# FAST-ASR/MarkovModels.jl

Hardware: AMD Instinct MI355X
Metric: pdfposteriors_frames_per_sec (higher is better)
Workload: dtype f32

## Files before the change

### markovmodels.jl_amd/csrc/mm_kernel_pairs.hip

```cpp
#pragma once
#include <algorithm>
#include "mm_internal.h"
#include "mm_kernel_rows.hip"

namespace mm {

typedef float mm_f32x2 __attribute__((ext_vector_type(2)));
typedef unsigned mm_u32x2 __attribute__((ext_vector_type(2)));
__device__ __forceinline__ mm_u32x2 ldsr2u(unsigned addr) { return *(__attribute__((address_space(3))) const mm_u32x2 *)(__UINTPTR_TYPE__)addr; }
__device__ __forceinline__ mm_f32x2 ldsr2(unsigned addr) { return *(__attribute__((address_space(3))) const mm_f32x2 *)(__UINTPTR_TYPE__)addr; }
__device__ __forceinline__ void ldsw2(unsigned addr, float a, float b) {
    mm_f32x2 v = {a, b};
    *(__attribute__((address_space(3))) mm_f32x2 *)(__UINTPTR_TYPE__)addr = v;
}

constexpr int pair_pc(int NJ) { return NJ > 4 ? 64 * NJ : 256; }
constexpr int pair_nr(int RS, int PC) { return (PC > 256 || RS > 16384) ? 2 : 3; }
template <int RS, int PHASE, int RSH = 2 * RS, int PC = 256>
struct PairLay {
    static constexpr unsigned RS2 = 2 * RS;
    static constexpr unsigned PC4 = 4u * PC, PC8 = 8u * PC;
    static constexpr int NR = pair_nr(RS, PC);
    static constexpr unsigned RAWS = 2u * PC4;
    static constexpr unsigned XPS = 2u * PC;
    static constexpr unsigned PP(int par) { return unsigned(par) * RS2; }
    static constexpr unsigned RAW(int k, int u) { return 2 * RS2 + unsigned(2 * k + u) * PC4; }
    static constexpr unsigned EM(int par) { return 2 * RS2 + 8u * PC4 + unsigned(par) * PC8; }
    static constexpr unsigned MS(int par) { return 2 * RS2 + 8u * PC4 + 2u * PC8 + unsigned(par) * 64u; }
    static constexpr unsigned OWN(int k) { return 2 * RS2 + 8u * PC4 + 2u * PC8 + 128u + unsigned(k) * 16u; }
    static constexpr unsigned XFLAG = 2 * RS2 + 8u * PC4 + 2u * PC8 + 192u;
    static constexpr unsigned MX(int par) { return 2 * RS2 + 8u * PC4 + 2u * PC8 + 200u + unsigned(par) * 8u; }
    static constexpr int POFFN = NR == 2 ? 4 : 8;
    static constexpr unsigned POFFB = 16u * POFFN;
    static constexpr unsigned POFF(int k, int u) { return 2 * RS2 + 8u * PC4 + 2u * PC8 + 256u + unsigned(2 * k + u) * 8u; }
    static constexpr unsigned PSUM(int par) { return 2 * RS2 + 8u * PC4 + 2u * PC8 + 256u + POFFB + unsigned(par) * PC8; }
    static constexpr unsigned PDFSE = 2 * RS2 + 8u * PC4 + 4u * PC8 + 256u + POFFB;
    static constexpr unsigned FIX = PDFSE + PC4;
    static constexpr unsigned AL(int k) { return FIX + unsigned(k) * RSH; }
    static constexpr unsigned Q(int par) { return FIX + unsigned(NR) * RSH + unsigned(par) * RSH; }
    static constexpr unsigned SLOTS = PHASE ? FIX + unsigned(NR + 2) * RSH : FIX;
};
inline size_t pair_lds_bytes(int RS, int phase, int nslotrows, int RSH = 0, int PC = 256) {
    const size_t fix = size_t(4 * RS) + size_t(8 * 4 * PC) + size_t(4 * 8 * PC) + 256 + (pair_nr(RS, PC) == 2 ? 64 : 128) + size_t(4 * PC);
    return fix + (phase ? size_t(pair_nr(RS, PC) + 2) * size_t(RSH ? RSH : 2 * RS) : 0) + size_t(nslotrows) * 64 * 8;
}

typedef unsigned long long mm_u64;
typedef __attribute__((address_space(1))) mm_u64 mm_gu64;
#ifndef MM_SPLIT_TIMEOUT
#ifndef MM_PAIR_LINFIN
#define MM_PAIR_LINFIN 1
#endif
#ifndef MM_PAIR_SCAN_BATCH
#define MM_PAIR_SCAN_BATCH 8
#endif
#define MM_LINF_EMIN (-40.f)
#define MM_SPLIT_TIMEOUT 10000000ull
#endif
__device__ __forceinline__ void granule_store(float *base, unsigned byte_off, float a, float b) {
    const mm_u64 v = ((mm_u64)__builtin_bit_cast(unsigned, b) << 32) | __builtin_bit_cast(unsigned, a);
    __hip_atomic_store((mm_gu64 *)(__UINTPTR_TYPE__)(reinterpret_cast<char *>(base) + byte_off), v, __ATOMIC_RELAXED, __HIP_MEMORY_SCOPE_AGENT);
}
__device__ __forceinline__ mm_u64 granule_load(const float *base, unsigned byte_off) {
    return __hip_atomic_load((mm_gu64 *)(__UINTPTR_TYPE__)(reinterpret_cast<const char *>(base) + byte_off), __ATOMIC_RELAXED,
                             __HIP_MEMORY_SCOPE_AGENT);
}
// ... 154 lines not shown
        "v_max_f32_dpp %1, %1, %1 row_mirror row_mask:0xf bank_mask:0xf\n\ts_nop 1"
        : "+v"(a), "+v"(b));
    const int ia = __builtin_bit_cast(int, a), ib = __builtin_bit_cast(int, b);
    const float a0 = __builtin_bit_cast(float, __builtin_amdgcn_readlane(ia, 0)), b0 = __builtin_bit_cast(float, __builtin_amdgcn_readlane(ib, 0));
    const float a1 = __builtin_bit_cast(float, __builtin_amdgcn_readlane(ia, 16)), b1 = __builtin_bit_cast(float, __builtin_amdgcn_readlane(ib, 16));
    const float a2 = __builtin_bit_cast(float, __builtin_amdgcn_readlane(ia, 32)), b2 = __builtin_bit_cast(float, __builtin_amdgcn_readlane(ib, 32));
    const float a3 = __builtin_bit_cast(float, __builtin_amdgcn_readlane(ia, 48)), b3 = __builtin_bit_cast(float, __builtin_amdgcn_readlane(ib, 48));
    a = fmaxf(fmaxf(a0, a1), fmaxf(a2, a3));
    b = fmaxf(fmaxf(b0, b1), fmaxf(b2, b3));
}

__device__ __forceinline__ float wave_max_of2(float a, float b) {
    float v = max_nc(a, b);
    asm("s_nop 1\n\tv_max_f32_dpp %0, %0, %0 quad_perm:[1,0,3,2] row_mask:0xf bank_mask:0xf\n\ts_nop 1\n\t"
        "v_max_f32_dpp %0, %0, %0 quad_perm:[2,3,0,1] row_mask:0xf bank_mask:0xf\n\ts_nop 1\n\t"
        "v_max_f32_dpp %0, %0, %0 row_half_mirror row_mask:0xf bank_mask:0xf\n\ts_nop 1\n\t"
        "v_max_f32_dpp %0, %0, %0 row_mirror row_mask:0xf bank_mask:0xf\n\ts_nop 1\n\t"
        "v_max_f32_dpp %0, %0, %0 row_bcast:15 row_mask:0xa bank_mask:0xf\n\ts_nop 1\n\t"
        "v_max_f32_dpp %0, %0, %0 row_bcast:31 row_mask:0xc bank_mask:0xf\n\ts_nop 1"
        : "+v"(v));
    return __builtin_bit_cast(float, __builtin_amdgcn_readlane(__builtin_bit_cast(int, v), 63));
}

template <int NJ, bool ADAPT>
__device__ __forceinline__ void pair_stage_em2(unsigned dst, unsigned raw0, unsigned raw1, int n, int len0, int len1, int P, int lane, float S0,
                                               float S1, float (&E)[2], float &X, int *mark0, int *mark1) {
    float v0[NJ], v1[NJ];
#pragma unroll
    for (int j = 0; j < NJ; ++j) {
        v0[j] = ldsr(raw0 + 256u * j + 4u * lane);
        v1[j] = ldsr(raw1 + 256u * j + 4u * lane);
    }
    float e0 = MM_NINF, e1 = MM_NINF;
#pragma unroll
    for (int j = 0; j < NJ; ++j) {
        const int q = lane + 64 * j;
        v0[j] = em_value(v0[j], n, len0, P, q);
        v1[j] = em_value(v1[j], n, len1, P, q);
        if (q < P) {
            e0 = max_nc(e0, v0[j]);
            e1 = max_nc(e1, v1[j]);
        }
    }
    wave_max_rl2(e0, e1);
    if (!(e0 > MM_NINF)) e0 = 0.f;
    if (!(e1 > MM_NINF)) e1 = 0.f;
    float n0 = 0.f, n1 = 0.f;
#pragma unroll
    for (int j = 0; j < NJ; ++j) {
        const int q = lane + 64 * j;
        if (q <= P) {
            const float x0 = v0[j] - e0 - S0, x1 = v1[j] - e1 - S1;
            ldsw2(dst + 8u * (unsigned)q, fast_exp2(x0), fast_exp2(x1));
            n0 = max_nc(n0, v0[j] > MM_NINF ? -x0 : 0.f);
            n1 = max_nc(n1, v1[j] > MM_NINF ? -x1 : 0.f);
        }
    }
    if constexpr (ADAPT) {
        X = wave_max_of2(n0, n1);
    } else {
        if (n0 > -MM_LINF_EMIN) *mark0 = 1;
        if (n1 > -MM_LINF_EMIN) *mark1 = 1;
    }
    E[0] = e0;
    E[1] = e1;
}

template <int NJ, bool LIN = false>
__device__ __forceinline__ void pair_stage_em_wide(unsigned dst, unsigned raw0, unsigned raw1, int n, int len0, int len1, int P, int lane,
                                                   float (&E)[2], float S0 = 0.f, float S1 = 0.f, int *mark0 = nullptr, int *mark1 = nullptr) {
    constexpr int NP = (NJ + 3) / 4;
    mm_f32x4 v0[NP], v1[NP];
#pragma unroll
    for (int j = 0; j < NP; ++j) {
        const unsigned o = 4u * (unsigned)(256 * j + 4 * lane);
        v0[j] = *(__attribute__((address_space(3))) const mm_f32x4 *)(__UINTPTR_TYPE__)(raw0 + o);
        v1[j] = *(__attribute__((address_space(3))) const mm_f32x4 *)(__UINTPTR_TYPE__)(raw1 + o);
    }
    float e0 = MM_NINF, e1 = MM_NINF;
#pragma unroll
    for (int j = 0; j < NP; ++j) {
#pragma unroll
        for (int i = 0; i < 4; ++i) {
            const int q = 256 * j + 4 * lane + i;
            v0[j][i] = em_value(v0[j][i], n, len0, P, q);
            v1[j][i] = em_value(v1[j][i], n, len1, P, q);
            if (q < P) {
                e0 = max_nc(e0, v0[j][i]);
// ... 324 lines not shown
#ifndef MM_PAIR_PRIO_A
#define MM_PAIR_PRIO_A 8
#define MM_PAIR_PRIO_B 16
#endif
#define MM_PAIR_PRIO(k, lvl) if constexpr (2 * (k) < KA) __builtin_amdgcn_s_setprio(lvl);
#define MM_PAIR_CASES(M)                                                                                     \
    M(0) M(2) M(4) M(6) MM_PAIR_PRIO(MM_PAIR_PRIO_A, 1) M(8) M(10) M(12)                                     \
    if (lastp >= 14) {                                                                                       \
        M(14) MM_PAIR_PRIO(MM_PAIR_PRIO_B, 0) M(16)                                                          \
        if (lastp >= 18) {                                                                                   \
            M(18)                                                                                            \
            if (lastp >= 20) { M(20) M(22) }                                                                 \
        }                                                                                                    \
    }

struct PairHand {
    float m_prev, s_cur, s_prev, cbar;
    int seen, pad;
    double cum;
};

template <int KA, int RS, int PHASE, int DIRT, int NJ, int H = 1, int RSH = 2 * RS, bool SMALL = false, bool XPT = false>
__device__ __forceinline__ void pair_agent(const RunParams &p, int pair, int hset = 0, int rdir = 0) {
#ifndef MM_SPLIT_MAXTRACK
#define MM_SPLIT_MAXTRACK 0
#endif
    extern __shared__ float lds[];
    const int DIR = DIRT < 0 ? __builtin_amdgcn_readfirstlane(rdir) : DIRT;
    const unsigned long long x_tmo = p.x_timeout;
    using L = PairLay<RS, PHASE, RSH, pair_pc(NJ)>;
#ifndef MM_PAIR_DA
#define MM_PAIR_DA 3
#endif
#ifndef MM_PAIR_DB
#define MM_PAIR_DB 3
#endif
#ifndef MM_PAIR_EXITS_B
#define MM_PAIR_EXITS_B 1
#endif
    constexpr bool MM_PAIR_DOUBLE = true;
    constexpr bool LINF = MM_PAIR_LINFIN != 0 && NJ <= 4;
    constexpr bool ADAPT = LINF && H == 1;
    constexpr int D = PHASE ? MM_PAIR_DB : MM_PAIR_DA;
    const int tid = threadIdx.x, NT = blockDim.x, lane = tid & 63;
    const int wave = __builtin_amdgcn_readfirstlane(tid >> 6), NW = NT >> 6, NWC = NW - (H > 1 ? 2 : 1);
    const bool service = wave == NWC;
    const bool xwave = H > 1 && wave == NWC + 1;
    if (service || xwave) __builtin_amdgcn_s_setprio(3);
    PairUtt U[2];
    int NFp = 1;
#pragma unroll
    for (int u = 0; u < 2; ++u) {
        const int i = 2 * pair + u;
// ... 12 lines not shown
    }
    static_assert(!XPT || PHASE == 0, "the export runs phase A");
    if constexpr (XPT) NFp = p.N + 1;
    float *rowsP = p.ws_alpha + (long long)pair * (long long)(p.N + 2) * 2 * p.pair_s1p;
    const UttDesc &ud = p.utts[U[0].b];
    const RowU r = uni(H > 1 ? ud.rps[DIR][hset] : ud.rp[DIR]);
    const int S1 = r.rows, S1p = p.pair_s1p, P1 = uni(ud.P1), P = P1 - 1, P1p = (P1 + 3) & ~3;
    const float thr = r.thr;
    unsigned sthr = 0u;
    if constexpr (LINF && !ADAPT)
        asm volatile("v_readfirstlane_b32 %0, %1" : "=s"(sthr) : "v"(((unsigned)(127 - (int)(thr + MM_LINF_EMIN < 1.f ? 1.f : thr + MM_LINF_EMIN)) << 23) - 1u));
    int m = (int)(((long long)NFp * (p.split_q10 > 0 ? p.split_q10 : 512)) >> 10);
    m = m < 1 ? 1 : (m > NFp - 1 && NFp > 1 ? NFp - 1 : m);
    const int tA = XPT ? NFp : (DIR ? NFp - m : m), tEnd = NFp;
    auto frame_of = [&](int t) { return DIR ? NFp + 1 - t : t; };
    PairHand *hand = reinterpret_cast<PairHand *>(p.pair_hand) + ((long long)pair * 2 + DIR) * 2;
    if (lds_addr_of(lds) != 0u) __builtin_trap();
    MM_STAMP_DECL;

    for (unsigned q = tid * 4u; q < 2u * L::RS2; q += NT * 4u) ldsw(L::PP(0) + q, 0.f);
    if constexpr (PHASE == 1)
        for (unsigned q = tid * 4u; q < 2u * RSH; q += NT * 4u) ldsw(L::Q(0) + q, 0.f);
    if (tid < 32) ldsw(L::MS(0) + 4u * tid, 0.f);
    if (tid < 4) ldswu(L::MX(0) + 4u * tid, 0u);
    if (tid < 4) ldsw(L::EM(tid >> 1) + 8u * P1p + 4u * (tid & 1), LINF ? 0.f : MM_NINF);
    const int nslotwords = r.nslotrows * 128;
    for (int q = tid; q < nslotwords; q += NT) ldswu(L::SLOTS + 4u * q, as_global(r.slots)[q]);
    if constexpr (PHASE == 1)
        for (int q = tid; q < P1; q += NT) ldswu(L::PDFSE + 4u * q, as_global(reinterpret_cast<const unsigned *>(r.pdfse))[q]);
    int *redo0 = p.redo + U[0].b, *redo1 = p.redo + (U[1].valid ? U[1].b : p.B);
    const int xbase = H > 1 ? p.sp_base[hset] : 0, xcnt = H > 1 ? p.sp_cnt[hset] : 0;
    float *xsend = nullptr, *xps_send = nullptr;
    bool xplain = false;
    const float *xrecv[H], *xps_recv[H];
    if constexpr (H > 1) {
        float *xb = p.xbuf + (long long)PHASE * p.x_phase + ((long long)pair * 2 + DIR) * H * 2 * p.x_slot;
        float *xq = p.xps + ((long long)pair * 2 + DIR) * H * 4 * (int)L::XPS;
#pragma unroll
        for (int g = 0; g < H; ++g) {
            xrecv[g] = g == hset ? nullptr : xb + (long long)g * 2 * p.x_slot;
            xps_recv[g] = g == hset ? nullptr : xq + (long long)g * 4 * (int)L::XPS;
        }
        xsend = xb + (long long)hset * 2 * p.x_slot;
        xps_send = xq + (long long)hset * 4 * (int)L::XPS;
    }
    unsigned long long endmask = 0, lgw0 = 0;
    int nslots = 0, start2 = 0;
// ... 55 lines not shown
#pragma unroll
            for (int u = 0; u < 2; ++u) row_dma_em<NJ>(L::RAW(0, u) + L::RAWS * (unsigned)(t & 3), U[u].Vb, p.vsn, frame_of(tt), p.N, P, sl);
        };
        auto dma_partner = [&](int t) {
            const int tt = t < 1 ? 1 : (t > tEnd ? tEnd : t);
            int f = frame_of(tt);
            f = f > p.N ? p.N : f;
            const int n4 = H > 1 ? (xcnt + 1) >> 1 : S1p >> 1;
            constexpr int NDM = RSH / 1024;
            const mm_f32x4 *src = reinterpret_cast<const mm_f32x4 *>(rowsP + (long long)f * 2 * S1p + 2 * xbase);
            const unsigned dst = L::AL(0) + (unsigned)(tt % L::NR) * (unsigned)RSH;
            if constexpr (small_graph) {
                dma_b128(src + (sl < n4 ? sl : 0), dst);
            } else {
                (void)n4;
                dma_row_b128<NDM>(uni(src), (unsigned)sl, dst);
            }
#pragma unroll
            for (int u = 0; u < 2; ++u)
                if (sl < 2) dma_b32(reinterpret_cast<const unsigned *>(U[u].offs + f) + sl, L::POFF(0, u) + 16u * (unsigned)(t & (L::POFFN - 1)));
        };
        constexpr int NDMA = 2 * NJ + (PHASE ? RSH / 1024 + 2 : 0);
        constexpr int NDMA_SMALL = 2 * NJ + (PHASE ? 1 + 2 : 0);
        auto stage = [&](int t, const float (&S)[2]) {
            float E[2], X = 0.f;
#ifndef MM_PAIR_WIDE_SERVICE
#define MM_PAIR_WIDE_SERVICE 1
#endif
            if constexpr (NJ > 4 && MM_PAIR_WIDE_SERVICE) {
                pair_stage_em_wide<NJ, LINF>(L::EM(t & 1), L::RAW(0, 0) + L::RAWS * (unsigned)(t & 3), L::RAW(0, 1) + L::RAWS * (unsigned)(t & 3), frame_of(t),
                                             U[0].len, U[1].len, P, sl, E, S[0], S[1], redo0, redo1);
            } else if constexpr (LINF) {
                pair_stage_em2<NJ, ADAPT>(L::EM(t & 1), L::RAW(0, 0) + L::RAWS * (unsigned)(t & 3), L::RAW(0, 1) + L::RAWS * (unsigned)(t & 3), frame_of(t),
                                          U[0].len, U[1].len, P, sl, S[0], S[1], E, X, redo0, redo1);
            } else {
#pragma unroll
                for (int u = 0; u < 2; ++u)
                    E[u] = pair_stage_em<NJ, LINF>(L::EM(t & 1), L::RAW(0, u) + L::RAWS * (unsigned)(t & 3), u, frame_of(t), U[u].len, P, sl, S[u], u ? redo1 : redo0);
            }
            double before[2];
#pragma unroll
            for (int u = 0; u < 2; ++u) {
                before[u] = cum[u];
                cum[u] += (double)S[u] + (double)E[u];
            }
            if constexpr (ADAPT) {
                float room = thr_v - X;
                if (room < 16.f) {
                    room = 16.f;
                    if (sl == 0) {
                        *redo0 = 1;
                        *redo1 = 1;
                    }
                }
// ... 21 lines not shown
                norm[u].s_prev = h.s_prev;
                norm[u].cbar = h.cbar;
                norm[u].seen = h.seen;
                cum[u] = h.cum;
            }
        }
        MM_ROW_VMCNT(0);
        if (PHASE == 0 || (DIR == 1 && !LINF)) {
            float E[2];
#pragma unroll
            for (int u = 0; u < 2; ++u) E[u] = pair_stage_em<NJ>(L::EM(t0 & 1), L::RAW(0, u) + L::RAWS * (unsigned)(t0 & 3), u, frame_of(t0), U[u].len, P, sl);
            if (PHASE == 0) {
#pragma unroll
                for (int u = 0; u < 2; ++u) cum[u] = (double)E[u];
                if (DIR == 0 && sl == 0) {
                    U[0].offs[1] = cum[0];
                    U[1].offs[1] = cum[1];
                }
            }
        }
        __syncthreads();
        if (t0 + 1 <= t1) {
            const float S[2] = {norm[0].s_cur, norm[1].s_cur};
            stage(t0 + 1, S);
        }
        dma_raw(t0 + 4);
        __syncthreads();
        const bool gwide = p.gsp == 1 && ((p.gsn | p.gsb) & 1) == 0 && ((__UINTPTR_TYPE__)p.gamma & 7) == 0;
        auto frames_of_step = [&](int ts, unsigned psum) {
            const int f = frame_of(ts);
            const bool live0 = f >= 1 && f <= U[0].len, live1 = f >= 1 && f <= U[1].len;
            float lt[2];
            const float *xp[H];
#pragma unroll
            for (int g = 0; g < H; ++g) xp[g] = (H > 1 && g != hset) ? xps_recv[g] + (ts & 3) * (int)L::XPS : nullptr;
            const bool writer = H == 1 || hset == 0;
            if constexpr (H == 1 && NJ > 4 && MM_PAIR_WIDE_SERVICE) {
                pair_finish_frames_wide<NJ>(psum, P1, P, sl, p.gamma + (long long)U[0].b * p.gsb + (long long)(f - 1) * p.gsn,
                                            p.gamma + (long long)U[1].b * p.gsb + (long long)(f - 1) * p.gsn, p.gsp, live0 && U[0].valid,
                                            live1 && U[1].valid, gwide, lt);
            } else if (!pair_finish_frames<NJ, H>(psum, P1, P, sl, p.gamma + (long long)U[0].b * p.gsb + (long long)(f - 1) * p.gsn,
                                           p.gamma + (long long)U[1].b * p.gsb + (long long)(f - 1) * p.gsn, p.gsp,
                                           live0 && U[0].valid && writer, live1 && U[1].valid && writer, lt, xp, split_tag(ts, t0, 2),
                                           xdead ? 0ull : x_tmo)) {
                if (sl == 0) {
                    *redo0 = 2;
                    *redo1 = 2;
// ... 4 lines not shown
            for (int u = 0; u < 2; ++u)
                if (u ? live1 : live0) {
                    const double own = *(__attribute__((address_space(3))) const double *)(__UINTPTR_TYPE__)(L::OWN(ts & 3) + 8u * u);
                    const double oth = *(__attribute__((address_space(3))) const double *)(__UINTPTR_TYPE__)(L::POFF(0, u) + 16u * (unsigned)(ts & (L::POFFN - 1)));
                    const double z = (double)lt[u] + own + oth;
                    zmin[u] = z < zmin[u] ? z : zmin[u];
                    zmax[u] = z > zmax[u] ? z : zmax[u];
                    if (!(z == z)) zmax[u] = __builtin_inf();
                    ltmin[u] = lt[u] < ltmin[u] ? lt[u] : ltmin[u];
                }
        };
        auto step = [&](auto RDc, int t) {
            constexpr int RD = decltype(RDc)::value, WR = 1 - RD;
#ifndef MM_PAIR_OPAQUE_B
#define MM_PAIR_OPAQUE_B 0
#endif
            if constexpr (H > 1 || NJ > 2 || (MM_PAIR_OPAQUE_B && PHASE == 1)) asm volatile("" : "+v"(sl));
            constexpr bool ring2 = PHASE == 1 && L::NR == 2;
            if constexpr (ring2) dma_partner(t + 1);
            else if constexpr (small_graph) asm volatile("s_waitcnt vmcnt(%0)" ::"n"(NDMA_SMALL) : "memory");
            else asm volatile("s_waitcnt vmcnt(%0)" ::"n"(NDMA) : "memory");
            MM_STAMP(2);
            float mx[2];
            if constexpr (H > 1 && MM_SPLIT_MAXTRACK) {
                if (t == t0 + 1) {
                    pair_scan_max<(RS / 8 + 63) / 64>(L::PP(RD), (S1 + 2) >> 1, sl, mx[0], mx[1]);
                } else {
                    const mm_u32x2 w = ldsr2u(L::MX(RD));
                    mx[0] = fast_log2(__builtin_bit_cast(float, (unsigned)__builtin_amdgcn_readfirstlane((int)w.x)));
                    mx[1] = fast_log2(__builtin_bit_cast(float, (unsigned)__builtin_amdgcn_readfirstlane((int)w.y)));
                }
                if (sl == 0) {
                    ldswu(L::MX(RD), 0u);
                    ldswu(L::MX(RD) + 4u, 0u);
                }
            } else if constexpr (small_graph) pair_scan_max<4>(L::PP(RD), (S1 + 2) >> 1, sl, mx[0], mx[1]);
            else pair_scan_max<(RS / 8 + 63) / 64, MM_PAIR_SCAN_BATCH>(L::PP(RD), (S1 + 2) >> 1, sl, mx[0], mx[1]);
            MM_STAMP(3);
            if (t + 1 <= tEnd) {
                const float S[2] = {norm[0].next(mx[0]), norm[1].next(mx[1])};
                if (t + 1 <= t1) stage(t + 1, S);
            }
            MM_STAMP(4);
            dma_raw(t + 4);
            if constexpr (PHASE == 1) {
                if constexpr (!ring2) dma_partner(t + 2);
                MM_STAMP(5);
                if constexpr (H == 1)
                    if (t - 2 > t0) frames_of_step(t - 2, L::PSUM(WR));
                MM_STAMP(6);
                if constexpr (ring2) asm volatile("s_waitcnt vmcnt(%0)" ::"n"(2 * NJ) : "memory");
                else if constexpr (small_graph) asm volatile("s_waitcnt vmcnt(%0)" ::"n"(NDMA_SMALL) : "memory");
                else asm volatile("s_waitcnt vmcnt(%0)" ::"n"(NDMA) : "memory");
                MM_STAMP(7);
            }
            MM_STAMP(0);
            MM_STEP_SYNC();
            MM_STAMP(1);
        };
        MM_STAMP_RESET;
        for (int t = t0 + 1; t <= t1; t += 2) {
            if (t & 1) step(std::integral_constant<int, 0>{}, t);
            else step(std::integral_constant<int, 1>{}, t);
            if (t + 1 <= t1) {
// ... 204 lines not shown
                const mm_f32x2 vv = *reinterpret_cast<const mm_f32x2 *>(rowsP + ((long long)f * S1p + i) * 2);
                float v0 = vv.x, v1 = vv.y;
                const unsigned pdfi = as_global(r.rowpdf)[i];
                if constexpr (LINF) {
                    if (H > 1 && pdfi == 0xffffu) v0 = v1 = 0.f;
                    ldsw2(L::PP(t0 & 1) + 8u * i, v0, v1);
                    continue;
                }
                if (DIR == 1) {
                    const mm_f32x2 e = ldsr2(L::EM(t0 & 1) + 8u * (H > 1 && pdfi == 0xffffu ? (unsigned)P1p : pdfi));
                    v0 += e.x;
                    v1 += e.y;
                }
                if (H > 1 && pdfi == 0xffffu) v0 = v1 = MM_NINF;
                ldsw2(L::PP(t0 & 1) + 8u * i, fast_exp2(v0), fast_exp2(v1));
            }
        }
        load_graph();
        __syncthreads();
        if constexpr (H > 1) xplain = __builtin_amdgcn_readfirstlane(ldsru(L::XFLAG)) != 0u;
        bool cdead = H > 1 && (p.x_sleep & 0x200) != 0;
        auto step = [&](auto RDc, int t) {
            constexpr int RD = decltype(RDc)::value, WR = 1 - RD;
            float vmx0 = 0.f, vmx1 = 0.f;
            if (nslots > 0) {
                constexpr unsigned rdoff = L::PP(RD);
                mm_f32x2 x[2 * D];
#pragma unroll
                for (int j = 0; j < D; ++j) {
                    x[2 * j] = ldsr2(rg.a[(2 * j < KA) ? 2 * j : 0] + rdoff);
                    x[2 * j + 1] = ldsr2(rg.a[(2 * j + 1 < KA) ? 2 * j + 1 : 0] + rdoff);
                }
                unsigned sa = slot_base;
                unsigned info, info2 = 0u, infoN, info2N = 0u;
                if constexpr (PHASE == 1) {
                    const mm_u32x2 w0 = ldsr2u(sa), w1 = ldsr2u(sa + 512u);
                    info = w0.x;
                    info2 = w0.y;
                    infoN = w1.x;
                    info2N = w1.y;
                } else {
                    info = ldsru(sa);
                    infoN = ldsru(sa + 512u);
                }
                mm_f32x2 S = {0.f, 0.f};
                if constexpr (!LINF) S = ldsr2(L::MS(WR));
                mm_f32x2 e = ldsr2((info >> 16) + L::EM(WR));
                const int f = frame_of(t);
                const unsigned alb = L::AL(0) + (unsigned)(t % L::NR) * (unsigned)RSH;
                mm_f32x2 al = {0.f, 0.f};
                float *xw = H > 1 ? xsend + (long long)(t & 1) * p.x_slot - 2 * xbase : nullptr;
                const float xsg = (H > 1 && split_tag(t, t0, 1)) ? -1.f : 1.f;
                if constexpr (PHASE == 1) al = ldsr2((info2 & 0xffffu) + alb);
                float *rowP = rowsP + (long long)(f <= p.N + (XPT ? 1 : 0) ? f : 0) * 2 * S1p;
                float worst = 0.f;
                unsigned smin = 0xffffffffu;
                mm_f32x2 accA = {0.f, 0.f}, accN = {0.f, 0.f};
                mm_f32x2 &accB = accA;
                unsigned long long lgw = lgw0;
                auto finish = [&]() {
                    const int lg = (int)(lgw & 15ull);
                    lgw >>= 4;
                    float s0 = accA.x, s1 = accA.y;
                    if (lg) grp_sum_last2(s0, s1, lg);
                    const unsigned pos8 = info & 0xffffu;
                    if constexpr (LINF) {
                        smin = min3_u32(smin, __builtin_bit_cast(unsigned, s0) - 1u, __builtin_bit_cast(unsigned, s1) - 1u);
                        mm_f32x2 sv = {s0, s1}, pv, qv;
                        asm("v_pk_mul_f32 %0, %1, %2" : "=v"(pv) : "v"(sv), "v"(e));
                        ldsw2(pos8 + L::PP(WR), pv.x, pv.y);
                        if constexpr (H > 1) {
                            if (xplain) *reinterpret_cast<mm_f32x2 *>(reinterpret_cast<char *>(xw) + pos8) = mm_f32x2{pv.x * xsg, pv.y * xsg};
                            else granule_store(xw, pos8, pv.x * xsg, pv.y * xsg);
                        }
                        if constexpr (PHASE == 0) {
                            if constexpr (XPT) *reinterpret_cast<mm_f32x2 *>(reinterpret_cast<char *>(rowP) + pos8) = DIR ? sv : pv;
                            else *reinterpret_cast<mm_f32x2 *>(reinterpret_cast<char *>(rowP) + pos8) = pv;
                        } else {
                            asm("v_pk_mul_f32 %0, %1, %2" : "=v"(qv) : "v"(sv), "v"(al));
                            ldsw2((info2 >> 16) + L::Q(WR), qv.x, qv.y);
                        }
                    } else {
                    const float b0 = fast_log2(s0) - S.x, b1 = fast_log2(s1) - S.y;
                    const float y0 = b0 + e.x, y1 = b1 + e.y;
                    worst = __builtin_fmaxf(worst, __builtin_fmaxf(__builtin_fmaf(__builtin_fabsf(y0), 0.f, __builtin_fabsf(y0)),
                                                                   __builtin_fmaf(__builtin_fabsf(y1), 0.f, __builtin_fabsf(y1))));
                    const float p0 = fast_exp2(y0), p1 = fast_exp2(y1);
                    ldsw2(pos8 + L::PP(WR), p0, p1);
                    if constexpr (H > 1 && MM_SPLIT_MAXTRACK) {
                        vmx0 = max_nc(vmx0, p0);
                        vmx1 = max_nc(vmx1, p1);
                    }
                    if constexpr (H > 1) {
                        if (xplain) *reinterpret_cast<mm_f32x2 *>(reinterpret_cast<char *>(xw) + pos8) = mm_f32x2{p0 * xsg, p1 * xsg};
                        else granule_store(xw, pos8, p0 * xsg, p1 * xsg);
                    }
                    const float st0 = DIR ? b0 : y0, st1 = DIR ? b1 : y1;
                    if constexpr (PHASE == 0) {
                        *reinterpret_cast<mm_f32x2 *>(reinterpret_cast<char *>(rowP) + pos8) = mm_f32x2{st0, st1};
                    } else {
                        ldsw2((info2 >> 16) + L::Q(WR), fast_exp2(st0 + al.x), fast_exp2(st1 + al.y));
                    }
                    }
                    accA = mm_f32x2{0.f, 0.f};
                    sa += 512u;
                    asm volatile("v_mov_b32 %0, %1" : "=v"(info) : "v"(infoN));
                    e = ldsr2((info >> 16) + L::EM(WR));
                    if constexpr (PHASE == 1) {
                        asm volatile("v_mov_b32 %0, %1" : "=v"(info2) : "v"(info2N));
                        al = ldsr2((info2 & 0xffffu) + alb);
                        const mm_u32x2 w1 = ldsr2u(sa + 512u);
                        infoN = w1.x;
                        info2N = w1.y;
                    } else {
                        infoN = ldsru(sa + 512u);
                    }
                };
                asm volatile("" : "+s"(em_lo), "+s"(em_hi));
                __builtin_amdgcn_s_setprio(2);
                MM_PAIR_CASES(MM_PAIR_TWO)
                if (__builtin_expect(__builtin_amdgcn_ballot_w64(LINF ? smin < (ADAPT ? ldsru(L::MS(WR)) : sthr) : worst > thr) != 0ull, 0)) {
                    *redo0 = 1;
                    *redo1 = 1;
                }
            }
            if constexpr (PHASE == 1)
                if (t - 1 > t0)
                    pair_pdf_sums<(NJ > 4 ? 1 : (NJ > 2 ? 2 : 3))>(L::Q(RD), L::PDFSE, L::PSUM(RD), P1, wave, NWC, lane, H > 1 ? xps_send + ((t - 1) & 3) * (int)L::XPS : nullptr,
                                  (H > 1 && split_tag(t - 1, t0, 2)) ? -1.f : 1.f);
            if constexpr (H > 1 && MM_SPLIT_CWPOLL) {
                constexpr int NG2 = (RSH / 16 + 63) / 64, I = (H - 1) * NG2;
                typedef unsigned mm_u32x4 __attribute__((ext_vector_type(4)));
                const unsigned tg = split_tag(t, t0, 1);
                if constexpr (H > 2) {
                    constexpr int NI = (I + 13) / 14;
                    static_assert(NI >= 2 && NI <= 4, "items per wave");
                    const float *srcs[NI];
                    unsigned offs2[NI], dst2[NI];
                    bool pnd[NI], sec[NI], any = false;
#pragma unroll
                    for (int e = 0; e < NI; ++e) {
                        const int i = wave + e * NWC, ic = i < I ? i : 0;
                        const int q = ic / NG2, j = ic % NG2, g = q < hset ? q : q + 1;
                        srcs[e] = uni(xrecv[g] + (long long)(t & 1) * p.x_slot);
                        const int ng = p.sp_cnt[g];
                        dst2[e] = L::PP(WR) + 8u * (unsigned)p.sp_base[g] + 16u * (unsigned)(lane + 64 * j);
                        pnd[e] = i < I && 2 * (lane + 64 * j) < ng;
// ... 13 lines not shown
                            else if constexpr (NI == 3)
                                asm volatile("global_load_dwordx4 %0, %3, %4 sc1\n\tglobal_load_dwordx4 %1, %5, %6 sc1\n\t"
                                             "global_load_dwordx4 %2, %7, %8 sc1\n\ts_waitcnt vmcnt(0)"
                                             : "=&v"(v[0]), "=&v"(v[1]), "=&v"(v[2])
                                             : "v"(offs2[0]), "s"(srcs[0]), "v"(offs2[1]), "s"(srcs[1]), "v"(offs2[2]), "s"(srcs[2])
                                             : "memory");
                            else
                                asm volatile("global_load_dwordx4 %0, %4, %5 sc1\n\tglobal_load_dwordx4 %1, %6, %7 sc1\n\t"
                                             "global_load_dwordx4 %2, %8, %9 sc1\n\tglobal_load_dwordx4 %3, %10, %11 sc1\n\ts_waitcnt vmcnt(0)"
                                             : "=&v"(v[0]), "=&v"(v[1]), "=&v"(v[2]), "=&v"(v[3])
                                             : "v"(offs2[0]), "s"(srcs[0]), "v"(offs2[1]), "s"(srcs[1]), "v"(offs2[2]), "s"(srcs[2]), "v"(offs2[3]),
                                               "s"(srcs[3])
                                             : "memory");
                            any = false;
#pragma unroll
                            for (int e = 0; e < NI; ++e) {
                                if (pnd[e] && (v[e].x >> 31) == tg && (!sec[e] || (v[e].z >> 31) == tg)) {
                                    mm_f32x4 w;
                                    w.x = __builtin_bit_cast(float, v[e].x & 0x7fffffffu);
                                    w.y = __builtin_bit_cast(float, v[e].y & 0x7fffffffu);
                                    w.z = sec[e] ? __builtin_bit_cast(float, v[e].z & 0x7fffffffu) : 0.f;
                                    w.w = sec[e] ? __builtin_bit_cast(float, v[e].w & 0x7fffffffu) : 0.f;
                                    *(__attribute__((address_space(3))) mm_f32x4 *)(__UINTPTR_TYPE__)dst2[e] = w;
                                    vmx0 = max_nc(vmx0, max_nc(w.x, w.z));
                                    vmx1 = max_nc(vmx1, max_nc(w.y, w.w));
                                    pnd[e] = false;
                                }
                                any = any || pnd[e];
                            }
                            if (__builtin_amdgcn_ballot_w64(any) == 0ull) break;
                            if (__builtin_amdgcn_s_memrealtime() - tstart > x_tmo) {
                                cdead = true;
                                if (lane == 0) {
                                    *redo0 = 2;
                                    *redo1 = 2;
                                }
                                break;
                            }
                            __builtin_amdgcn_s_sleep(1);
                        }
                    }
                } else
                for (int i = wave; i < I; i += NWC) {
                    const int q = i / NG2, j = i % NG2, g = q < hset ? q : q + 1;
                    const float *src = xrecv[g] + (long long)(t & 1) * p.x_slot;
                    const int ng = p.sp_cnt[g];
                    const unsigned dsta = L::PP(WR) + 8u * (unsigned)p.sp_base[g] + 16u * (unsigned)(lane + 64 * j);
                    const bool have = 2 * (lane + 64 * j) < ng, second = 2 * (lane + 64 * j) + 1 < ng;
                    const unsigned off = have ? 16u * (unsigned)(lane + 64 * j) : 0u;
                    bool pend = have;
                    if (__builtin_amdgcn_ballot_w64(pend) == 0ull || cdead) continue;
                    const unsigned long long tstart = __builtin_amdgcn_s_memrealtime();
                    for (;;) {
                        mm_u32x4 v;
                        asm volatile("global_load_dwordx4 %0, %1, %2 sc1\n\ts_waitcnt vmcnt(0)" : "=v"(v) : "v"(off), "s"(src) : "memory");
                        if (pend && (v.x >> 31) == tg && (!second || (v.z >> 31) == tg)) {
                            mm_f32x4 w;
                            w.x = __builtin_bit_cast(float, v.x & 0x7fffffffu);
                            w.y = __builtin_bit_cast(float, v.y & 0x7fffffffu);
                            w.z = second ? __builtin_bit_cast(float, v.z & 0x7fffffffu) : 0.f;
                            w.w = second ? __builtin_bit_cast(float, v.w & 0x7fffffffu) : 0.f;
                            *(__attribute__((address_space(3))) mm_f32x4 *)(__UINTPTR_TYPE__)dsta = w;
                            vmx0 = max_nc(vmx0, max_nc(w.x, w.z));
                            vmx1 = max_nc(vmx1, max_nc(w.y, w.w));
                            pend = false;
                        }
                        if (__builtin_amdgcn_ballot_w64(pend) == 0ull) break;
                        if (__builtin_amdgcn_s_memrealtime() - tstart > x_tmo) {
                            cdead = true;
                            if (lane == 0) {
                                *redo0 = 2;
                                *redo1 = 2;
                            }
                            break;
                        }
                        __builtin_amdgcn_s_sleep(1);
                    }
                }
            }
            if constexpr (H > 1 && MM_SPLIT_MAXTRACK) {
                const float m0 = wave_max_rl(vmx0), m1 = wave_max_rl(vmx1);
                if (lane == 0) {
                    typedef __attribute__((address_space(3))) unsigned lds_u32;
                    (void)__hip_atomic_fetch_max((lds_u32 *)(__UINTPTR_TYPE__)L::MX(WR), __builtin_bit_cast(unsigned, m0), __ATOMIC_RELAXED,
                                                 __HIP_MEMORY_SCOPE_WORKGROUP);
                    (void)__hip_atomic_fetch_max((lds_u32 *)(__UINTPTR_TYPE__)(L::MX(WR) + 4u), __builtin_bit_cast(unsigned, m1), __ATOMIC_RELAXED,
                                                 __HIP_MEMORY_SCOPE_WORKGROUP);
                }
            }
            MM_STAMP(0);
            MM_STEP_SYNC();
            MM_STAMP(1);
        };
        MM_STAMP_RESET;
        for (int t = t0 + 1; t <= t1; t += 2) {
            if (t & 1) step(std::integral_constant<int, 0>{}, t);
            else step(std::integral_constant<int, 1>{}, t);
            if (t + 1 <= t1) {
                if ((t + 1) & 1) step(std::integral_constant<int, 0>{}, t + 1);
                else step(std::integral_constant<int, 1>{}, t + 1);
            }
        }
        if constexpr (PHASE == 1) {
            if (t1 > t0)
                pair_pdf_sums<(NJ > 4 ? 1 : (NJ > 2 ? 2 : 3))>(L::Q(t1 & 1), L::PDFSE, L::PSUM(t1 & 1), P1, wave, NWC, lane, H > 1 ? xps_send + (t1 & 3) * (int)L::XPS : nullptr,
                              (H > 1 && split_tag(t1, t0, 2)) ? -1.f : 1.f);
            __syncthreads();
        }
    }
#ifdef MM_STAMPS
// ... 146 lines not shown
```

### markovmodels.jl_amd/csrc/mm_pairs_tu.hip

```cpp
#define MM_SECONDARY_TU
#include "mm_internal.h"
#include "mm_kernel_pairs.hip"

namespace mm {

template <int NJ, int PHASE, bool SMALL>
__global__ void __launch_bounds__(1024) mm_fbp_kernel(RunParams p) {
    const int npairs = (p.B + 1) / 2, dir = (int)blockIdx.x >= npairs;
    pair_agent<MM_PAIR_KA, MM_ROW_RS, PHASE, -1, NJ, 1, 2 * MM_ROW_RS, SMALL>(p, (int)blockIdx.x - (dir ? npairs : 0), 0, dir);
}
template <int NJ, int PHASE, bool SMALL>
static int launch_pair_phase(const PairLaunch &pl, const RunParams &p, hipStream_t st) {
    return pair_launch_phase(mm_fbp_kernel<NJ, PHASE, SMALL>, "pair kernel", pair_lds_bytes(MM_ROW_RS, PHASE, pl.slotrows, 0, pair_pc(NJ)),
                             2 * pair_count(pl), pl.nwc + 1, st, p);
}
template <int NJ, bool SMALL>
static int launch_pairs_ka(const PairLaunch &pl, const RunParams &p, hipStream_t s0) {
    return pair_launch_phases(launch_pair_phase<NJ, 0, SMALL>, launch_pair_phase<NJ, 1, SMALL>, mm_pair_finish_kernel, pl, p, s0);
}
int mm_launch_pairs(const PairLaunch &pl, const RunParams &p, hipStream_t s0) {
    if (pl.pair_ka > MM_PAIR_KA) return MM_ERR_UNSUPPORTED;
    if (pl.max_P1 <= 128) return pl.small ? launch_pairs_ka<2, true>(pl, p, s0) : launch_pairs_ka<2, false>(pl, p, s0);
    if (pl.max_P1 <= 250) return launch_pairs_ka<4, false>(pl, p, s0);
    if (pl.max_P1 > MM_PAIR_P1MAX) return MM_ERR_UNSUPPORTED;
    return launch_pairs_ka<8, false>(pl, p, s0);
}
template <int NJ, bool SMALL>
__global__ void __launch_bounds__(1024) mm_fbx_kernel(RunParams p, int dir) {
    pair_agent<MM_PAIR_KA, MM_ROW_RS, 0, -1, NJ, 1, 2 * MM_ROW_RS, SMALL, true>(p, (int)blockIdx.x, 0, dir);
}
template <int NJ, bool SMALL>
static int launch_pair_export(const PairLaunch &pl, const RunParams &p, int dir, hipStream_t st) {
    const int rc = pair_launch_phase(mm_fbx_kernel<NJ, SMALL>, "pair kernel", pair_lds_bytes(MM_ROW_RS, 0, pl.slotrows, 0, pair_pc(NJ)), pair_count(pl),
                                     pl.nwc + 1, st, p, dir);
    return rc ? rc : pair_launch_export_layout(pl, p, dir, st);
}
bool mm_pair_export_fits(const PairLaunch &pl) { return pl.H == 1 && pl.pair_ka <= MM_PAIR_KA && pl.max_P1 <= 250; }
int mm_launch_pair_export(const PairLaunch &pl, const RunParams &p, int dir, hipStream_t s0) {
    if (!mm_pair_export_fits(pl)) return MM_ERR_UNSUPPORTED;
    if (pl.max_P1 <= 128) return pl.small ? launch_pair_export<2, true>(pl, p, dir, s0) : launch_pair_export<2, false>(pl, p, dir, s0);
    return launch_pair_export<4, false>(pl, p, dir, s0);
}
size_t mm_pair_lds_bytes(int phase, int nslotrows, int max_P1) {
    return pair_lds_bytes(MM_ROW_RS, phase, nslotrows, 0, pair_pc(mm_pair_nj(max_P1)));
}
size_t mm_pair_hand_bytes() { return sizeof(PairHand); }

}
```

Baseline: 148.6 million.

## Track per-step maxima in an LDS table and prefetch emission reads early

Replaces the per-step full scan of the previous probability row (pair_scan_max) with a 512-byte-per-parity LDS maxima table. Producers update the table with atomic fetch_max as they write new values, and consumers reduce it with one wave reduction. It also splits the emission staging into read, max and put steps, so the raw emission loads and max reduction can be issued before the scan wait and overlap it. This adds LDS atomics in the inner loop and 1 KB of LDS, and disables the table for the wide phase-1 case.

```diff
diff --git a/markovmodels.jl_amd/csrc/mm_kernel_pairs.hip b/markovmodels.jl_amd/csrc/mm_kernel_pairs.hip
--- a/markovmodels.jl_amd/csrc/mm_kernel_pairs.hip
+++ b/markovmodels.jl_amd/csrc/mm_kernel_pairs.hip
@@ -16,7 +16,8 @@
 
 constexpr int pair_pc(int NJ) { return NJ > 4 ? 64 * NJ : 256; }
 constexpr int pair_nr(int RS, int PC) { return (PC > 256 || RS > 16384) ? 2 : 3; }
-template <int RS, int PHASE, int RSH = 2 * RS, int PC = 256>
+constexpr bool pair_mxt(int NJ, int phase) { return !(NJ > 4 && phase == 1); }
+template <int RS, int PHASE, int RSH = 2 * RS, int PC = 256, bool MXT = false>
 struct PairLay {
     static constexpr unsigned RS2 = 2 * RS;
     static constexpr unsigned PC4 = 4u * PC, PC8 = 8u * PC;
@@ -29,19 +30,23 @@
     static constexpr unsigned MS(int par) { return 2 * RS2 + 8u * PC4 + 2u * PC8 + unsigned(par) * 64u; }
     static constexpr unsigned OWN(int k) { return 2 * RS2 + 8u * PC4 + 2u * PC8 + 128u + unsigned(k) * 16u; }
     static constexpr unsigned XFLAG = 2 * RS2 + 8u * PC4 + 2u * PC8 + 192u;
-    static constexpr unsigned MX(int par) { return 2 * RS2 + 8u * PC4 + 2u * PC8 + 200u + unsigned(par) * 8u; }
+    static constexpr unsigned MXB = MXT ? 1024u : 0u;
+    static constexpr unsigned MX(int par) {
+        static_assert(MXT, "this layout has no maxima table");
+        return 2 * RS2 + 8u * PC4 + 4u * PC8 + 256u + POFFB + PC4 + unsigned(par) * 512u;
+    }
     static constexpr int POFFN = NR == 2 ? 4 : 8;
     static constexpr unsigned POFFB = 16u * POFFN;
     static constexpr unsigned POFF(int k, int u) { return 2 * RS2 + 8u * PC4 + 2u * PC8 + 256u + unsigned(2 * k + u) * 8u; }
     static constexpr unsigned PSUM(int par) { return 2 * RS2 + 8u * PC4 + 2u * PC8 + 256u + POFFB + unsigned(par) * PC8; }
     static constexpr unsigned PDFSE = 2 * RS2 + 8u * PC4 + 4u * PC8 + 256u + POFFB;
-    static constexpr unsigned FIX = PDFSE + PC4;
+    static constexpr unsigned FIX = PDFSE + PC4 + MXB;
     static constexpr unsigned AL(int k) { return FIX + unsigned(k) * RSH; }
     static constexpr unsigned Q(int par) { return FIX + unsigned(NR) * RSH + unsigned(par) * RSH; }
     static constexpr unsigned SLOTS = PHASE ? FIX + unsigned(NR + 2) * RSH : FIX;
 };
-inline size_t pair_lds_bytes(int RS, int phase, int nslotrows, int RSH = 0, int PC = 256) {
-    const size_t fix = size_t(4 * RS) + size_t(8 * 4 * PC) + size_t(4 * 8 * PC) + 256 + (pair_nr(RS, PC) == 2 ? 64 : 128) + size_t(4 * PC);
+inline size_t pair_lds_bytes(int RS, int phase, int nslotrows, int RSH = 0, int PC = 256, bool mxt = false) {
+    const size_t fix = size_t(4 * RS) + size_t(8 * 4 * PC) + size_t(4 * 8 * PC) + 256 + (pair_nr(RS, PC) == 2 ? 64 : 128) + size_t(4 * PC) + (mxt ? 1024 : 0);
     return fix + (phase ? size_t(pair_nr(RS, PC) + 2) * size_t(RSH ? RSH : 2 * RS) : 0) + size_t(nslotrows) * 64 * 8;
 }
 
@@ -242,15 +247,16 @@
     return __builtin_bit_cast(float, __builtin_amdgcn_readlane(__builtin_bit_cast(int, v), 63));
 }
 
-template <int NJ, bool ADAPT>
-__device__ __forceinline__ void pair_stage_em2(unsigned dst, unsigned raw0, unsigned raw1, int n, int len0, int len1, int P, int lane, float S0,
-                                               float S1, float (&E)[2], float &X, int *mark0, int *mark1) {
-    float v0[NJ], v1[NJ];
+template <int NJ>
+__device__ __forceinline__ void pair_em2_read(unsigned raw0, unsigned raw1, int lane, float (&v0)[NJ], float (&v1)[NJ]) {
 #pragma unroll
     for (int j = 0; j < NJ; ++j) {
         v0[j] = ldsr(raw0 + 256u * j + 4u * lane);
         v1[j] = ldsr(raw1 + 256u * j + 4u * lane);
     }
+}
+template <int NJ>
+__device__ __forceinline__ void pair_em2_max(float (&v0)[NJ], float (&v1)[NJ], int n, int len0, int len1, int P, int lane, float (&E)[2]) {
     float e0 = MM_NINF, e1 = MM_NINF;
 #pragma unroll
     for (int j = 0; j < NJ; ++j) {
@@ -265,6 +271,13 @@
     wave_max_rl2(e0, e1);
     if (!(e0 > MM_NINF)) e0 = 0.f;
     if (!(e1 > MM_NINF)) e1 = 0.f;
+    E[0] = e0;
+    E[1] = e1;
+}
+template <int NJ, bool ADAPT>
+__device__ __forceinline__ void pair_em2_put(unsigned dst, const float (&v0)[NJ], const float (&v1)[NJ], int P, int lane, float S0, float S1,
+                                             const float (&E)[2], float &X, int *mark0, int *mark1) {
+    const float e0 = E[0], e1 = E[1];
     float n0 = 0.f, n1 = 0.f;
 #pragma unroll
     for (int j = 0; j < NJ; ++j) {
@@ -282,8 +295,14 @@
         if (n0 > -MM_LINF_EMIN) *mark0 = 1;
         if (n1 > -MM_LINF_EMIN) *mark1 = 1;
     }
-    E[0] = e0;
-    E[1] = e1;
+}
+template <int NJ, bool ADAPT>
+__device__ __forceinline__ void pair_stage_em2(unsigned dst, unsigned raw0, unsigned raw1, int n, int len0, int len1, int P, int lane, float S0,
+                                               float S1, float (&E)[2], float &X, int *mark0, int *mark1) {
+    float v0[NJ], v1[NJ];
+    pair_em2_read<NJ>(raw0, raw1, lane, v0, v1);
+    pair_em2_max<NJ>(v0, v1, n, len0, len1, P, lane, E);
+    pair_em2_put<NJ, ADAPT>(dst, v0, v1, P, lane, S0, S1, E, X, mark0, mark1);
 }
 
 template <int NJ, bool LIN = false>
@@ -654,13 +673,14 @@
 
 template <int KA, int RS, int PHASE, int DIRT, int NJ, int H = 1, int RSH = 2 * RS, bool SMALL = false, bool XPT = false>
 __device__ __forceinline__ void pair_agent(const RunParams &p, int pair, int hset = 0, int rdir = 0) {
-#ifndef MM_SPLIT_MAXTRACK
-#define MM_SPLIT_MAXTRACK 0
+#ifndef MM_PAIR_MXFIN_A
+#define MM_PAIR_MXFIN_A 0
 #endif
     extern __shared__ float lds[];
     const int DIR = DIRT < 0 ? __builtin_amdgcn_readfirstlane(rdir) : DIRT;
     const unsigned long long x_tmo = p.x_timeout;
-    using L = PairLay<RS, PHASE, RSH, pair_pc(NJ)>;
+    constexpr bool MXTAB = H == 1 && pair_mxt(NJ, PHASE);
+    using L = PairLay<RS, PHASE, RSH, pair_pc(NJ), MXTAB>;
 #ifndef MM_PAIR_DA
 #define MM_PAIR_DA 3
 #endif
@@ -719,7 +739,8 @@
     if constexpr (PHASE == 1)
         for (unsigned q = tid * 4u; q < 2u * RSH; q += NT * 4u) ldsw(L::Q(0) + q, 0.f);
     if (tid < 32) ldsw(L::MS(0) + 4u * tid, 0.f);
-    if (tid < 4) ldswu(L::MX(0) + 4u * tid, 0u);
+    if constexpr (MXTAB)
+        for (unsigned q = tid * 4u; q < L::MXB; q += NT * 4u) ldswu(L::MX(0) + q, 0u);
     if (tid < 4) ldsw(L::EM(tid >> 1) + 8u * P1p + 4u * (tid & 1), LINF ? 0.f : MM_NINF);
     const int nslotwords = r.nslotrows * 128;
     for (int q = tid; q < nslotwords; q += NT) ldswu(L::SLOTS + 4u * q, as_global(r.slots)[q]);
@@ -821,7 +842,9 @@
         };
         constexpr int NDMA = 2 * NJ + (PHASE ? RSH / 1024 + 2 : 0);
         constexpr int NDMA_SMALL = 2 * NJ + (PHASE ? 1 + 2 : 0);
-        auto stage = [&](int t, const float (&S)[2]) {
+        constexpr bool EMPRE = H == 1 && LINF;
+        float em_v0[NJ], em_v1[NJ], em_E[2] = {0.f, 0.f};
+        auto stage = [&](int t, const float (&S)[2], auto pre) {
             float E[2], X = 0.f;
 #ifndef MM_PAIR_WIDE_SERVICE
 #define MM_PAIR_WIDE_SERVICE 1
@@ -829,6 +852,10 @@
             if constexpr (NJ > 4 && MM_PAIR_WIDE_SERVICE) {
                 pair_stage_em_wide<NJ, LINF>(L::EM(t & 1), L::RAW(0, 0) + L::RAWS * (unsigned)(t & 3), L::RAW(0, 1) + L::RAWS * (unsigned)(t & 3), frame_of(t),
                                              U[0].len, U[1].len, P, sl, E, S[0], S[1], redo0, redo1);
+            } else if constexpr (EMPRE && decltype(pre)::value) {
+                E[0] = em_E[0];
+                E[1] = em_E[1];
+                pair_em2_put<NJ, ADAPT>(L::EM(t & 1), em_v0, em_v1, P, sl, S[0], S[1], E, X, redo0, redo1);
             } else if constexpr (LINF) {
                 pair_stage_em2<NJ, ADAPT>(L::EM(t & 1), L::RAW(0, 0) + L::RAWS * (unsigned)(t & 3), L::RAW(0, 1) + L::RAWS * (unsigned)(t & 3), frame_of(t),
                                           U[0].len, U[1].len, P, sl, S[0], S[1], E, X, redo0, redo1);
@@ -896,7 +923,7 @@
         __syncthreads();
         if (t0 + 1 <= t1) {
             const float S[2] = {norm[0].s_cur, norm[1].s_cur};
-            stage(t0 + 1, S);
+            stage(t0 + 1, S, std::false_type{});
         }
         dma_raw(t0 + 4);
         __syncthreads();
@@ -947,24 +974,30 @@
             else asm volatile("s_waitcnt vmcnt(%0)" ::"n"(NDMA) : "memory");
             MM_STAMP(2);
             float mx[2];
-            if constexpr (H > 1 && MM_SPLIT_MAXTRACK) {
+            if constexpr (EMPRE)
+                pair_em2_read<NJ>(L::RAW(0, 0) + L::RAWS * (unsigned)((t + 1) & 3), L::RAW(0, 1) + L::RAWS * (unsigned)((t + 1) & 3), sl, em_v0, em_v1);
+            if constexpr (MXTAB) {
                 if (t == t0 + 1) {
-                    pair_scan_max<(RS / 8 + 63) / 64>(L::PP(RD), (S1 + 2) >> 1, sl, mx[0], mx[1]);
+                    if constexpr (EMPRE) pair_em2_max<NJ>(em_v0, em_v1, frame_of(t + 1), U[0].len, U[1].len, P, sl, em_E);
+                    pair_scan_max<(small_graph ? 4 : (RS / 8 + 63) / 64), 4>(L::PP(RD), (S1 + 2) >> 1, sl, mx[0], mx[1]);
                 } else {
-                    const mm_u32x2 w = ldsr2u(L::MX(RD));
-                    mx[0] = fast_log2(__builtin_bit_cast(float, (unsigned)__builtin_amdgcn_readfirstlane((int)w.x)));
-                    mx[1] = fast_log2(__builtin_bit_cast(float, (unsigned)__builtin_amdgcn_readfirstlane((int)w.y)));
-                }
-                if (sl == 0) {
-                    ldswu(L::MX(RD), 0u);
-                    ldswu(L::MX(RD) + 4u, 0u);
-                }
-            } else if constexpr (small_graph) pair_scan_max<4>(L::PP(RD), (S1 + 2) >> 1, sl, mx[0], mx[1]);
-            else pair_scan_max<(RS / 8 + 63) / 64, MM_PAIR_SCAN_BATCH>(L::PP(RD), (S1 + 2) >> 1, sl, mx[0], mx[1]);
+                    const mm_u32x2 w = ldsr2u(L::MX(RD) + 8u * (unsigned)sl);
+                    if constexpr (EMPRE) pair_em2_max<NJ>(em_v0, em_v1, frame_of(t + 1), U[0].len, U[1].len, P, sl, em_E);
+                    const unsigned wa = w.x, wb = w.y;
+                    float a = __builtin_bit_cast(float, wa), b = __builtin_bit_cast(float, wb);
+                    wave_max_rl2(a, b);
+                    mx[0] = fast_log2(a);
+                    mx[1] = fast_log2(b);
+                }
+                *(__attribute__((address_space(3))) mm_u32x2 *)(__UINTPTR_TYPE__)(L::MX(RD) + 8u * (unsigned)sl) = mm_u32x2{0u, 0u};
+            } else {
+                static_assert(!EMPRE, "the linear instances of one workgroup have the table");
+                pair_scan_max<(RS / 8 + 63) / 64, MM_PAIR_SCAN_BATCH>(L::PP(RD), (S1 + 2) >> 1, sl, mx[0], mx[1]);
+            }
             MM_STAMP(3);
             if (t + 1 <= tEnd) {
                 const float S[2] = {norm[0].next(mx[0]), norm[1].next(mx[1])};
-                if (t + 1 <= t1) stage(t + 1, S);
+                if (t + 1 <= t1) stage(t + 1, S, std::true_type{});
             }
             MM_STAMP(4);
             dma_raw(t + 4);
@@ -1215,7 +1248,17 @@
         bool cdead = H > 1 && (p.x_sleep & 0x200) != 0;
         auto step = [&](auto RDc, int t) {
             constexpr int RD = decltype(RDc)::value, WR = 1 - RD;
+            constexpr bool MXFIN = MM_PAIR_MXFIN_A ? true : PHASE == 1;
+            typedef __attribute__((address_space(3))) unsigned lds_u32;
+            auto mx_post = [&](float m0, float m1, unsigned lane8) {
+                if constexpr (MXTAB) {
+                    lds_u32 *const mp = (lds_u32 *)(__UINTPTR_TYPE__)(L::MX(WR) + lane8);
+                    (void)__hip_atomic_fetch_max(mp, __builtin_bit_cast(unsigned, m0), __ATOMIC_RELAXED, __HIP_MEMORY_SCOPE_WORKGROUP);
+                    (void)__hip_atomic_fetch_max(mp + 1, __builtin_bit_cast(unsigned, m1), __ATOMIC_RELAXED, __HIP_MEMORY_SCOPE_WORKGROUP);
+                }
+            };
             float vmx0 = 0.f, vmx1 = 0.f;
+            (void)vmx0, (void)vmx1, (void)mx_post;
             if (nslots > 0) {
                 constexpr unsigned rdoff = L::PP(RD);
                 mm_f32x2 x[2 * D];
@@ -1262,6 +1305,12 @@
                         mm_f32x2 sv = {s0, s1}, pv, qv;
                         asm("v_pk_mul_f32 %0, %1, %2" : "=v"(pv) : "v"(sv), "v"(e));
                         ldsw2(pos8 + L::PP(WR), pv.x, pv.y);
+                        if constexpr (MXTAB && MXFIN) {
+                            mx_post(max_nc(pv.x, 0.f), max_nc(pv.y, 0.f), (sa - L::SLOTS) & 511u);
+                        } else if constexpr (MXTAB) {
+                            vmx0 = max_nc(vmx0, pv.x);
+                            vmx1 = max_nc(vmx1, pv.y);
+                        }
                         if constexpr (H > 1) {
                             if (xplain) *reinterpret_cast<mm_f32x2 *>(reinterpret_cast<char *>(xw) + pos8) = mm_f32x2{pv.x * xsg, pv.y * xsg};
                             else granule_store(xw, pos8, pv.x * xsg, pv.y * xsg);
@@ -1280,7 +1329,7 @@
                                                                    __builtin_fmaf(__builtin_fabsf(y1), 0.f, __builtin_fabsf(y1))));
                     const float p0 = fast_exp2(y0), p1 = fast_exp2(y1);
                     ldsw2(pos8 + L::PP(WR), p0, p1);
-                    if constexpr (H > 1 && MM_SPLIT_MAXTRACK) {
+                    if constexpr (MXTAB && !MXFIN) {
                         vmx0 = max_nc(vmx0, p0);
                         vmx1 = max_nc(vmx1, p1);
                     }
@@ -1316,6 +1365,7 @@
                     *redo0 = 1;
                     *redo1 = 1;
                 }
+                if constexpr (MXTAB && !MXFIN) mx_post(vmx0, vmx1, 8u * (unsigned)lane);
             }
             if constexpr (PHASE == 1)
                 if (t - 1 > t0)
@@ -1375,8 +1425,6 @@
                                     w.z = sec[e] ? __builtin_bit_cast(float, v[e].z & 0x7fffffffu) : 0.f;
                                     w.w = sec[e] ? __builtin_bit_cast(float, v[e].w & 0x7fffffffu) : 0.f;
                                     *(__attribute__((address_space(3))) mm_f32x4 *)(__UINTPTR_TYPE__)dst2[e] = w;
-                                    vmx0 = max_nc(vmx0, max_nc(w.x, w.z));
-                                    vmx1 = max_nc(vmx1, max_nc(w.y, w.w));
                                     pnd[e] = false;
                                 }
                                 any = any || pnd[e];
@@ -1414,8 +1462,6 @@
                             w.z = second ? __builtin_bit_cast(float, v.z & 0x7fffffffu) : 0.f;
                             w.w = second ? __builtin_bit_cast(float, v.w & 0x7fffffffu) : 0.f;
                             *(__attribute__((address_space(3))) mm_f32x4 *)(__UINTPTR_TYPE__)dsta = w;
-                            vmx0 = max_nc(vmx0, max_nc(w.x, w.z));
-                            vmx1 = max_nc(vmx1, max_nc(w.y, w.w));
                             pend = false;
                         }
                         if (__builtin_amdgcn_ballot_w64(pend) == 0ull) break;
@@ -1429,16 +1475,6 @@
                         }
                         __builtin_amdgcn_s_sleep(1);
                     }
-                }
-            }
-            if constexpr (H > 1 && MM_SPLIT_MAXTRACK) {
-                const float m0 = wave_max_rl(vmx0), m1 = wave_max_rl(vmx1);
-                if (lane == 0) {
-                    typedef __attribute__((address_space(3))) unsigned lds_u32;
-                    (void)__hip_atomic_fetch_max((lds_u32 *)(__UINTPTR_TYPE__)L::MX(WR), __builtin_bit_cast(unsigned, m0), __ATOMIC_RELAXED,
-                                                 __HIP_MEMORY_SCOPE_WORKGROUP);
-                    (void)__hip_atomic_fetch_max((lds_u32 *)(__UINTPTR_TYPE__)(L::MX(WR) + 4u), __builtin_bit_cast(unsigned, m1), __ATOMIC_RELAXED,
-                                                 __HIP_MEMORY_SCOPE_WORKGROUP);
                 }
             }
             MM_STAMP(0);
diff --git a/markovmodels.jl_amd/csrc/mm_pairs_tu.hip b/markovmodels.jl_amd/csrc/mm_pairs_tu.hip
--- a/markovmodels.jl_amd/csrc/mm_pairs_tu.hip
+++ b/markovmodels.jl_amd/csrc/mm_pairs_tu.hip
@@ -11,7 +11,7 @@
 }
 template <int NJ, int PHASE, bool SMALL>
 static int launch_pair_phase(const PairLaunch &pl, const RunParams &p, hipStream_t st) {
-    return pair_launch_phase(mm_fbp_kernel<NJ, PHASE, SMALL>, "pair kernel", pair_lds_bytes(MM_ROW_RS, PHASE, pl.slotrows, 0, pair_pc(NJ)),
+    return pair_launch_phase(mm_fbp_kernel<NJ, PHASE, SMALL>, "pair kernel", pair_lds_bytes(MM_ROW_RS, PHASE, pl.slotrows, 0, pair_pc(NJ), pair_mxt(NJ, PHASE)),
                              2 * pair_count(pl), pl.nwc + 1, st, p);
 }
 template <int NJ, bool SMALL>
@@ -31,7 +31,7 @@
 }
 template <int NJ, bool SMALL>
 static int launch_pair_export(const PairLaunch &pl, const RunParams &p, int dir, hipStream_t st) {
-    const int rc = pair_launch_phase(mm_fbx_kernel<NJ, SMALL>, "pair kernel", pair_lds_bytes(MM_ROW_RS, 0, pl.slotrows, 0, pair_pc(NJ)), pair_count(pl),
+    const int rc = pair_launch_phase(mm_fbx_kernel<NJ, SMALL>, "pair kernel", pair_lds_bytes(MM_ROW_RS, 0, pl.slotrows, 0, pair_pc(NJ), true), pair_count(pl),
                                      pl.nwc + 1, st, p, dir);
     return rc ? rc : pair_launch_export_layout(pl, p, dir, st);
 }
@@ -42,7 +42,8 @@
     return launch_pair_export<4, false>(pl, p, dir, s0);
 }
 size_t mm_pair_lds_bytes(int phase, int nslotrows, int max_P1) {
-    return pair_lds_bytes(MM_ROW_RS, phase, nslotrows, 0, pair_pc(mm_pair_nj(max_P1)));
+    const int nj = mm_pair_nj(max_P1);
+    return pair_lds_bytes(MM_ROW_RS, phase, nslotrows, 0, pair_pc(nj), pair_mxt(nj, phase));
 }
 size_t mm_pair_hand_bytes() { return sizeof(PairHand); }
 
```

Result: slower. 146.6 million (-1.3%).
